# Kolkir/feature-point-cnn

Measured on AMD Instinct MI355X. Metric: frames/sec (VGA 640x480) SuperPoint fwd+NMS+descriptors, higher is better.
Workload: dtype f32

## Files before the change

### experiments/harness/w36_bench.hip

```cpp
#include <hip/hip_runtime.h>
#include <stdint.h>
#include <cmath>
#include <cstdio>
#include <cstdlib>
#include <cstring>
#include <random>
#include <vector>
#include <algorithm>
#include "../../feature-point-cnn_amd/csrc/wblock36_mfma.h"
using namespace fpc;
#define CK(x) do { hipError_t e_ = (x); if (e_ != hipSuccess) { printf("HIP error %s at line %d\n", hipGetErrorString(e_), __LINE__); exit(1);} } while (0)

static const double G43[6][3] = {{1.0 / 4, 0, 0}, {-1.0 / 6, -1.0 / 6, -1.0 / 6}, {-1.0 / 6, 1.0 / 6, -1.0 / 6},
                                 {1.0 / 24, 1.0 / 12, 1.0 / 6}, {1.0 / 24, -1.0 / 12, 1.0 / 6}, {0, 0, 1}};

struct Problem {
  int B, H, W, Cin, N, Cx;
  bool conv_only; int ysplit;
};

template <int NB, int TYT, int TXT>
static double run(const Problem& P, bool check, int reps, int grid_override = 0) {
  using C = W36Cfg<NB, TYT, TXT>;
  const int N = C::N, ncg = N / 16, nchunk = P.Cin / 16, nout = P.conv_only ? N * P.ysplit : N;
// ... 39 lines not shown
  float *dx, *dw1, *dw2, *db2, *dout;
  const size_t nout_el = (size_t)P.B * P.H * P.W * nout;
  CK(hipMalloc(&dx, x.size() * 4)); CK(hipMalloc(&dw1, w1p.size() * 4)); CK(hipMalloc(&dw2, w2p.size() * 4));
  CK(hipMalloc(&db2, N * 4)); CK(hipMalloc(&dout, nout_el * 4));
  CK(hipMemcpy(dx, x.data(), x.size() * 4, hipMemcpyHostToDevice));
  CK(hipMemcpy(dw1, w1p.data(), w1p.size() * 4, hipMemcpyHostToDevice));
  CK(hipMemcpy(dw2, w2p.data(), w2p.size() * 4, hipMemcpyHostToDevice));
  CK(hipMemcpy(db2, b2.data(), N * 4, hipMemcpyHostToDevice));
  CK(hipMemset(dout, 0xff, nout_el * 4));
  if (getenv("W36_PTRS")) printf("x %p..%p  w1 %p..%p  w2 %p..%p  b2 %p  out %p..%p\n", dx, dx + x.size(), dw1, dw1 + w1p.size(), dw2, dw2 + w2p.size(), db2, dout, dout + nout_el);
  WBlockArgs a{};
  a.x = dx; a.csx = P.Cin; a.nchunk = nchunk; a.H = P.H; a.W = P.W;
  a.w1 = (const float4*)dw1; a.b1 = dw1 + (size_t)ncg * gstride; a.w2 = (const float4*)dw2; a.b2 = db2;
  a.k8_h = k8_h; a.k8_x = k8_x; a.out = dout; a.cso = nout;
  a.tiles_x = (P.W + C::TW - 1) / C::TW; a.tiles_y = (P.H + C::TH - 1) / C::TH; a.frame0 = 0;
  a.total = a.tiles_x * a.tiles_y * P.B; a.xcd_order = 1; a.ysplit_floats = (int)half_floats;
  a.x_bytes = (unsigned)(x.size() * 4); a.conv_only = P.conv_only ? 1 : 0;
#ifdef FPC_DIAG
  unsigned long long* dst_; CK(hipMalloc(&dst_, 1024 * 8 * 8 + 1024 * 4 * 16 * 8)); CK(hipMemset(dst_, 0, 1024 * 8 * 8 + 1024 * 4 * 16 * 8)); a.stamps = dst_;
#endif
  CK(hipFuncSetAttribute((const void*)wblock36_kernel<NB, TYT, TXT>, hipFuncAttributeMaxDynamicSharedMemorySize, C::LDS_BYTES));
  int grid = grid_override ? grid_override : 256;
  if (grid > a.total) grid = a.total >= 8 ? (a.total / 8) * 8 : a.total;
  const dim3 g(grid, nh);
  hipLaunchKernelGGL((wblock36_kernel<NB, TYT, TXT>), g, dim3(256), C::LDS_BYTES, 0, a);
  CK(hipDeviceSynchronize());
  double result = 0;
  if (check) {
    std::vector<float> out(nout_el);
    CK(hipMemcpy(out.data(), dout, nout_el * 4, hipMemcpyDeviceToHost));
// ... 123 lines not shown
```

### experiments/harness/w36p_bench.hip

```cpp
#include <hip/hip_runtime.h>
#include <stdint.h>
#include <cmath>
#include <cstdio>
#include <cstdlib>
#include <cstring>
#include <random>
#include <vector>
#include <algorithm>
#include "../../feature-point-cnn_amd/csrc/wblock36p_mfma.h"
using namespace fpc;
#ifndef W36P_RING
#define W36P_RING 9
#endif
#define CK(x) do { hipError_t e_ = (x); if (e_ != hipSuccess) { printf("HIP error %s at line %d\n", hipGetErrorString(e_), __LINE__); exit(1);} } while (0)

static const double G43[6][3] = {{1.0 / 4, 0, 0}, {-1.0 / 6, -1.0 / 6, -1.0 / 6}, {-1.0 / 6, 1.0 / 6, -1.0 / 6},
                                 {1.0 / 24, 1.0 / 12, 1.0 / 6}, {1.0 / 24, -1.0 / 12, 1.0 / 6}, {0, 0, 1}};

struct Problem {
  int B, H, W, Cin, N, Cx;
  bool conv_only; int ysplit;
};

template <int NBP, int TYT, int TXT>
// ... 52 lines not shown
  float *dx, *dw1, *dw2, *db2, *dout;
  const size_t nout_el = (size_t)P.B * P.H * P.W * nout;
  CK(hipMalloc(&dx, x.size() * 4)); CK(hipMalloc(&dw1, w1p.size() * 4)); CK(hipMalloc(&dw2, w2p.size() * 4));
  CK(hipMalloc(&db2, N * 4)); CK(hipMalloc(&dout, nout_el * 4));
  CK(hipMemcpy(dx, x.data(), x.size() * 4, hipMemcpyHostToDevice));
  CK(hipMemcpy(dw1, w1p.data(), w1p.size() * 4, hipMemcpyHostToDevice));
  CK(hipMemcpy(dw2, w2p.data(), w2p.size() * 4, hipMemcpyHostToDevice));
  CK(hipMemcpy(db2, b2.data(), N * 4, hipMemcpyHostToDevice));
  CK(hipMemset(dout, 0xff, nout_el * 4));
  if (getenv("W36_PTRS")) printf("x %p..%p  w1 %p..%p  w2 %p..%p  b2 %p  out %p..%p\n", dx, dx + x.size(), dw1, dw1 + w1p.size(), dw2, dw2 + w2p.size(), db2, dout, dout + nout_el);
  WBlockArgs a{};
  a.x = dx; a.csx = P.Cin; a.nchunk = nchunk; a.H = P.H; a.W = P.W;
  a.w1 = (const float4*)dw1; a.b1 = dw1 + (size_t)ncg * gstride; a.w2 = (const float4*)dw2; a.b2 = db2;
  a.k8_h = k8_h; a.k8_x = k8_x; a.out = dout; a.cso = nout;
  a.tiles_x = (P.W + C::TW - 1) / C::TW; a.tiles_y = (P.H + C::TH - 1) / C::TH; a.frame0 = 0;
  a.total = a.tiles_x * a.tiles_y * P.B; a.xcd_order = 1; a.ysplit_floats = (int)half_floats;
  a.x_bytes = (unsigned)(x.size() * 4); a.conv_only = P.conv_only ? 1 : 0;
#ifdef FPC_DIAG
  unsigned long long* dst_; CK(hipMalloc(&dst_, 1024 * 8 * 8 + 1024 * 4 * 16 * 8)); CK(hipMemset(dst_, 0, 1024 * 8 * 8 + 1024 * 4 * 16 * 8)); a.stamps = dst_;
#endif
  CK(hipFuncSetAttribute(fn, hipFuncAttributeMaxDynamicSharedMemorySize, LDSB));
  int grid = grid_override ? grid_override : 256;
  if (grid > a.total) grid = a.total >= 8 ? (a.total / 8) * 8 : a.total;
  const dim3 g(grid, nh);
  launch(g, a);
  CK(hipDeviceSynchronize());
  double result = 0;
  if (check) {
    std::vector<float> out(nout_el);
    CK(hipMemcpy(out.data(), dout, nout_el * 4, hipMemcpyDeviceToHost));
// ... 120 lines not shown
```

### feature-point-cnn_amd/_lib.py

```python
import ctypes
import os
import subprocess

import torch

_DIR = os.path.dirname(os.path.abspath(__file__))
LIB_PATH = os.environ.get("FPC_LIB_PATH") or os.path.join(_DIR, "lib", "libfpc.so")
CSRC = os.path.join(_DIR, "csrc")

SYMBOLS = [
    "fpc_abi_version", "fpc_build_flags", "fpc_strerror", "fpc_last_hip_error", "fpc_default_config", "fpc_create",
    "fpc_destroy", "fpc_load_weights", "fpc_packed_size", "fpc_packed_device_ptr",
    "fpc_export_packed", "fpc_import_packed", "fpc_import_packed_device", "fpc_mark_weights_loaded", "fpc_set_stream", "fpc_upload_stream",
    "fpc_get_stream", "fpc_sync", "fpc_forward", "fpc_detect", "fpc_get_points", "fpc_results",
    "fpc_get_counts", "fpc_get_keypoints", "fpc_set_timing", "fpc_get_timings", "fpc_match", "fpc_first_within",
    "fpc_detect_u8", "fpc_u8_staging", "fpc_homography_adaptation", "fpc_detect_u8_resized",
    "fpc_sample_descriptors", "fpc_plan_hash", "fpc_broadcast_weights", "fpc_read_activation",
    "fpc_pack_layout_revision", "fpc_check_guards", "fpc_stream_report", "fpc_output_range",
    "fpc_match_frames", "fpc_first_within_frames",
    "fpc_default_ransac_params", "fpc_ransac_homography", "fpc_homography_frames",
    "fpc_bank_create", "fpc_bank_destroy", "fpc_bank_get", "fpc_bank_store", "fpc_bank_store_rows", "fpc_bank_clear",
    "fpc_match_bank", "fpc_homography_bank", "fpc_bank_create_ex", "fpc_bank_format",
    "fpc_match_frames_guided", "fpc_match_bank_guided",
    "fpc_cell_order", "fpc_match_frames_guided_cells", "fpc_match_bank_guided_cells",
    "fpc_bank_topk_reserve", "fpc_match_bank_topk", "fpc_homography_bank_topk",
    "fpc_ransac_fundamental", "fpc_fundamental_frames", "fpc_fundamental_bank",
    "fpc_match_frames_guided_epipolar", "fpc_match_bank_guided_epipolar",
]

ABI_VERSION = 4
PACK_LAYOUT_REVISION = 4

PLAN_FLAGS = {
    "no_fused_blocks": 1 << 0, "no_winograd": 1 << 1, "no_winograd_detector": 1 << 2, "no_winograd_layer_in1": 1 << 3,
    "no_xcd_order": 1 << 4, "no_fused_stem_pool": 1 << 5, "split_heads": 1 << 6, "nms_in_line": 1 << 7,
    "no_persistent_grid": 1 << 8, "layer1_tile_8x16": 1 << 9, "winograd_gen1": 1 << 10, "no_latency_tiles": 1 << 11,
    "nms_one_workgroup": 1 << 12, "no_fused_softmax": 1 << 13, "winograd_gen2": 1 << 14, "guard_zones": 1 << 15, "detector_gen1": 1 << 16, "heads_in_line": 1 << 17, "w36_one_wave": 1 << 18, "convt_phases": 1 << 19, "stem_round3": 1 << 20, "conv_round1": 1 << 21,
}


class FpcConfig(ctypes.Structure):
    _fields_ = [("device", ctypes.c_int), ("height", ctypes.c_int), ("width", ctypes.c_int),
                ("max_batch", ctypes.c_int), ("cell", ctypes.c_int), ("nms_dist", ctypes.c_int),
                ("conf_thresh", ctypes.c_float), ("border_remove", ctypes.c_int),
                ("descriptor_enabled", ctypes.c_int), ("max_keypoints", ctypes.c_int),
                ("in_channels", ctypes.c_int), ("dtype", ctypes.c_int), ("arch", ctypes.c_int),
                ("num_streams", ctypes.c_int), ("plan_flags", ctypes.c_uint), ("nms_round_launches", ctypes.c_int),
                ("min_sub_batch", ctypes.c_int)]


class FpcTensor(ctypes.Structure):
    _fields_ = [("name", ctypes.c_char_p), ("data", ctypes.c_void_p), ("ndim", ctypes.c_int),
# ... 159 lines not shown
```

### feature-point-cnn_amd/csrc/fpc_api.hip

```cpp
#include <hip/hip_runtime.h>

#include <dlfcn.h>

#include <algorithm>
#include <cmath>
#include <cstdio>
#include <cstdlib>
#include <cstring>
#include <memory>
#include <mutex>
#include <chrono>
#include <string>
#include <vector>

#include "../../include/fpc.h"
#include "block_mfma.h"
#include "block_bf16.h"
#include "convt_bf16.h"
#include "block_x3.h"
#include "stem_bf16.h"
#include "wblock_mfma.h"
#include "wblock16_mfma.h"
#include "wblock36_mfma.h"
#include "wblock36p_mfma.h"
// ... 281 lines not shown
   W36PCfg<TYT, TXT, true>::LDS_BYTES, 4, 4 * TYT, 4 * TXT, 512, (const void*)wblock36p_dust_kernel<TYT, TXT>, launchw_##name, true},
    FPC_W36PD_KINDS(X)
#undef X
};

static size_t w1_floats(const WKindInfo& k, int nchunk) {
  if (k.gen == 3) return (size_t)k.NCG * ((size_t)nchunk * 36 + (k.NCG == 8 ? W36Cfg<2, 4, 4>::WPAD : W36Cfg<1, 4, 4>::WPAD)) * 256;
  return (size_t)k.NCG * ((size_t)nchunk * 16 + W16Cfg<8>::WPAD) * 256;
}
static double wkind_mfma_flops(const WKindInfo& k, int tiles, int nchunk, int k8_1x1) {
  const double px = (double)k.TH * k.TW, n = k.NBT * 32.0;
  if (k.gen == 3) return 2.0 * tiles * n * (36.0 * (px / 16) * nchunk * k.KC + px * k8_1x1 * 8.0);
  return 2.0 * tiles * n * (16.0 * (px / 4) * nchunk * k.KC + px * k8_1x1 * 8.0);
}
static bool w36_fits(int , int H, int W, int cs_in, int cs_out) {
  return (unsigned long long)H * W * (unsigned long long)std::max(cs_in, cs_out) * sizeof(float) < (unsigned long long)W36_MARKER;
}
static int w36_frames_per_launch(int H, int W, int cs_in, int cs_out) {
  const unsigned long long fb = (unsigned long long)H * W * (unsigned long long)std::max(cs_in, cs_out) * sizeof(float);
  return (int)std::max<unsigned long long>(1, ((unsigned long long)W36_MARKER - 1) / fb);
}
static int w36_conv_part(int cout, int tiles, int cus) {
  if (cout < 128) return 64;
  if (cout == 128) return 128;
  const double t2 = std::ceil((double)tiles * (cout / 128) / cus) * 1.0, t1 = std::ceil((double)tiles * (cout / 64) / cus) * 0.53;
  return t1 < t2 ? 64 : 128;
}
static WKind w36_kind(int cout, int H, int W, bool paired = false) {
  const int t44 = ((H + 15) / 16) * ((W + 15) / 16), t28 = ((H + 7) / 8) * ((W + 31) / 32);
  if (cout == 65 && paired) return t28 < t44 ? WK_W36PD_C65_2x8 : WK_W36PD_C65_4x4;
  if (cout == 65) return t28 < t44 ? WK_W36_C65_2x8 : WK_W36_C65_4x4;
// ... 94 lines not shown
  int pH = 0, pW = 0, pC = 0;
  std::string prefix;
  int cin = 0, cout = 0;
  int grid_y = 1, grid_z = 1;
  double flops_per_frame = 0;
  double mfma_flops_per_frame = 0;
  bool fused_softmax_capable = false;
  double bytes_per_frame = 0;
  bool descriptor_branch = false;
};

struct Timing {
  hipEvent_t start, stop;
  int op;
  int frames;
};

}

using namespace fpc;

struct fpc_ctx {
  fpc_config cfg{};
  int H = 0, W = 0, B = 0, Hc = 0, Wc = 0;
  bool vgg = false;
  int D = 128;
  std::vector<float*> vbuf;
  size_t vconv0_off = 0;
  bool bf16 = false;
  bool split = false;
// ... 27 lines not shown
  bool nms_one_workgroup = false;
  int nms_g = 0;
  bool fuse_stem_pool = true;
  bool conv_lean = true;
  bool stem_lean = true;
  bool stem2 = false;
  bool layer1_t816 = false;
#ifdef FPC_DIAG
  unsigned long long* diag_stamps = nullptr;
  int diag_n = 0;
#endif
  bool winograd_in1 = true;
  bool winograd_det = true;
  int w36_cus = 0;
  bool w36_paired = true;
  bool winograd_det_gen3 = true;
  bool winograd = true;
  bool latency_tiles = true;
  int winograd_gen = 3;
  bool fuse_blocks = true;
  bool weights_loaded = false;
  bool plan_error = false;

  char* slab = nullptr;
  size_t slab_bytes = 0;
  bool guard_zones = false;
  std::vector<std::pair<size_t, size_t>> guards;
  float *stem_out, *x0, *h4, *x1, *x2, *h8, *x3, *cat, *dh, *dproj, *d0, *lg;
  float *h16, *y16a, *y16b, *lo_h, *lo0, *desc_map, *desc_in_nhwc;
  float* prob;
// ... 1823 lines not shown

struct Sub {
  int f0, n;
  bool small = false;
  bool fuse_softmax = false;
  hipStream_t st;
  hipStream_t side = nullptr;
  hipEvent_t ev_enc = nullptr, ev_det = nullptr;
};

struct LaunchTimer {
  fpc_ctx* c;
  int op;
  hipStream_t st;
  int frames;
  hipEvent_t s{}, e{};
  LaunchTimer(fpc_ctx* c_, int op_, hipStream_t st_, int frames_) : c(c_), op(op_), st(st_), frames(frames_) {
    if (c->timing) {
      s = next_event(c);
      e = next_event(c);
      hipEventRecord(s, st);
    }
  }
  ~LaunchTimer() {
    if (c->timing) {
      hipEventRecord(e, st);
      c->timings.push_back({s, e, op, frames});
    }
  }
};

static int op_index(const fpc_ctx* c, OpType t) {
  for (size_t i = 0; i < c->ops.size(); ++i)
    if (c->ops[i].type == t) return (int)i;
  return -1;
}

static void run_network(fpc_ctx* c, const float* frames, const Sub& sb0, int which, hipStream_t st) {
  Sub sb = sb0;
  sb.st = st;
  const int H = c->H, W = c->W, n = sb.n, f0 = sb.f0;
  for (size_t i = 0; i < c->ops.size(); ++i) {
// ... 78 lines not shown
      case OP_WBLOCK: {
        LaunchTimer t(c, (int)i, sb.st, n);
        WBlockArgs a = op.wargs;
        a.frame0 = f0;
#ifdef FPC_DIAG
        a.stamps = nullptr;
        if (const char* e = getenv("FPC_STAMP_OP"))
          if (op.name.find(e) != std::string::npos) {
            if (!c->diag_stamps) hipHostMalloc((void**)&c->diag_stamps, (size_t)65536 * 8 * sizeof(unsigned long long));
            memset(c->diag_stamps, 0, (size_t)65536 * 8 * sizeof(unsigned long long));
            a.stamps = c->diag_stamps;
            c->diag_n = a.tiles_x * a.tiles_y * n;
          }
#endif
        a.total = a.tiles_x * a.tiles_y * n;
        a.xcd_order = c->xcd_order ? 1 : 0;
        {
          const unsigned long long xb = (unsigned long long)(f0 + n) * a.H * a.W * a.csx * sizeof(float);
          a.x_bytes = xb > 0xfffffff0ull ? 0xfffffff0u : (unsigned)xb;
        }
        int grid = (c->persist_min_tiles > 0 && a.total >= c->persist_min_tiles * c->num_cus) ? c->num_cus : a.total;
        if (g_wkinds[op.wkind].gen == 3) {
          const int fpl = w36_frames_per_launch(a.H, a.W, a.csx, a.cso);
          const float* x0 = a.x;
          float* o0 = a.out;
          for (int g0 = 0; g0 < n; g0 += fpl) {
            const int gn = std::min(fpl, n - g0);
            a.frame0 = 0;
            a.x = x0 + (size_t)(f0 + g0) * a.H * a.W * a.csx;
            a.out = o0 + (size_t)(f0 + g0) * a.H * a.W * a.cso;
            a.total = a.tiles_x * a.tiles_y * gn;
            a.x_bytes = (unsigned)((unsigned long long)gn * a.H * a.W * a.csx * sizeof(float));
            const int cus_cap = c->w36_cus > 0 ? std::min(c->num_cus, c->w36_cus) : c->num_cus;
            const int cus8 = std::max(1, cus_cap / 8 / std::max(1, op.grid_y)), per_xcd = (a.total + 7) / 8;
            const int rounds = (per_xcd + cus8 - 1) / cus8;
            const int grid3 = 8 * std::min(cus8, (per_xcd + rounds - 1) / rounds);
            g_wkinds[op.wkind].launch(a, dim3(std::min(a.total, grid3), op.grid_y), sb.st);
          }
          break;
        }
        g_wkinds[op.wkind].launch(a, dim3(std::min(a.total, grid), op.grid_y), sb.st);
        break;
      }
      case OP_BLOCK: {
        LaunchTimer t(c, (int)i, sb.st, n);
        BlockArgs a = op.bargs;
        a.frame0 = f0;
#ifdef FPC_DIAG
        a.stamps = nullptr;
        if (const char* e = getenv("FPC_STAMP_OP"))
          if (op.name.find(e) != std::string::npos) {
            if (!c->diag_stamps) hipHostMalloc((void**)&c->diag_stamps, (size_t)65536 * 8 * sizeof(unsigned long long));
            memset(c->diag_stamps, 0, (size_t)65536 * 8 * sizeof(unsigned long long));
// ... 373 lines not shown
  const auto create_t0 = std::chrono::steady_clock::now();
  std::unique_lock<std::mutex> queue_lock(qmap::state().mu);
  const int probe_rounds0 = qmap::state().dev[cfg->device].rounds;
  c->stream = qmap::acquire(cfg->device, c.get(), SLOT_MAIN, true, qprobe, true);
  if (!c->stream) { qmap::release_owner(c.get()); g_hip_err = "hipStreamCreateWithFlags"; return FPC_E_HIP; }
  c->own_stream = true;
  {
    int nsub = cfg->num_streams > 0 ? std::min(8, cfg->num_streams) : (c->split ? 3 : 2);
    const unsigned pf = cfg->plan_flags;
    c->fuse_blocks = !(pf & FPC_PLAN_NO_FUSED_BLOCKS);
    c->guard_zones = (pf & FPC_PLAN_GUARD_ZONES) != 0;
    if (const char* e = getenv("FPC_GUARD_ZONES")) c->guard_zones = atoi(e) != 0;
    c->winograd_det_gen3 = !(pf & FPC_PLAN_DETECTOR_GEN1);
    c->w36_paired = !(pf & FPC_PLAN_W36_ONE_WAVE);
    if (const char* e = getenv("FPC_W36_PAIRED")) c->w36_paired = atoi(e) != 0;
    if (const char* e = getenv("FPC_W36_CUS")) c->w36_cus = std::max(0, atoi(e));
    if (const char* e = getenv("FPC_WINOGRAD_DET_GEN")) c->winograd_det_gen3 = atoi(e) >= 3;
    c->winograd = !(pf & FPC_PLAN_NO_WINOGRAD);
    c->winograd_det = !(pf & FPC_PLAN_NO_WINOGRAD_DETECTOR);
    c->winograd_in1 = !(pf & FPC_PLAN_NO_WINOGRAD_LAYER_IN1);
    c->xcd_order = !(pf & FPC_PLAN_NO_XCD_ORDER);
    c->fuse_stem_pool = !(pf & FPC_PLAN_NO_FUSED_STEM_POOL);
    c->stem_lean = !(pf & FPC_PLAN_STEM_ROUND3);
    c->conv_lean = !(pf & FPC_PLAN_CONV_ROUND1);
    if (const char* e = getenv("FPC_CONV_LEAN")) c->conv_lean = atoi(e) != 0;
    if (const char* e = getenv("FPC_STEM_LEAN")) c->stem_lean = atoi(e) != 0;
    c->split_heads = (pf & FPC_PLAN_SPLIT_HEADS) != 0;
    if (pf & FPC_PLAN_NO_PERSISTENT_GRID) c->persist_min_tiles = 0;
    c->layer1_t816 = (pf & FPC_PLAN_LAYER1_TILE_8x16) != 0;
    c->winograd_gen = (pf & FPC_PLAN_WINOGRAD_GEN1) ? 1 : (pf & FPC_PLAN_WINOGRAD_GEN2) ? 2 : 3;
// ... 1375 lines not shown
          case OP_CONV: k = op->lean ? lean_kind(op->kind)->symbol : g_kinds[op->kind].symbol; break;
          case OP_BLOCK: k = g_bkinds[op->bkind].symbol; break;
          case OP_WBLOCK: k = g_wkinds[op->wkind].symbol; break;
          case OP_BF16: k = g_fkinds[op->fkind].symbol; break;
          case OP_SOFTMAX: k = "softmax_d2s_kernel"; break;
          case OP_NMS: k = c->nms_one_workgroup ? "nms_rounds_kernel+nms_sort_kernel" : "nms_rounds_kernel+nms_finish_kernel+nms_chunk_sort_kernel+nms_merge_kernel"; break;
          case OP_DESC: k = "descriptor16_kernel"; break;
          case OP_VCONV0: k = "vgg_conv0_kernel"; break;
          case OP_POOL2: k = "maxpool2_kernel"; break;
          case OP_L2NORM: k = "l2norm256_kernel"; break;
        }
      kernels[i] = k;
    }
    if (ms) ms[i] = v;
    if (flops) flops[i] = op ? op->flops_per_frame * t.frames : 0.0;
    if (mfma_flops) mfma_flops[i] = op ? op->mfma_flops_per_frame * t.frames : 0.0;
    if (bytes) bytes[i] = op ? op->bytes_per_frame * t.frames : 0.0;
  }
  return n;
}

}
```

### feature-point-cnn_amd/csrc/wblock36_mfma.h

```cpp
#pragma once
#include <type_traits>
#include <utility>

#include "wblock16_mfma.h"

namespace fpc {

template <int... I, class F>
__device__ __forceinline__ void fpc_static_for_impl(std::integer_sequence<int, I...>, F&& f) {
  (f(std::integral_constant<int, I>{}), ...);
}
template <int N, class F>
__device__ __forceinline__ void fpc_static_for(F&& f) {
  fpc_static_for_impl(std::make_integer_sequence<int, N>{}, f);
}

struct W36Dust {
  static constexpr int W2ROW = 0, W2COL = 64, WPCOL = 144, B1 = 400, B2 = 401, UIN64 = 404, UIN = 448, UOUT = 448 + 4 * 36 * 16;
  static constexpr int floats(int nchunk) { return UOUT + nchunk * 36 * 16; }
};

template <int NB_, int TYT_, int TXT_, bool DUST_ = false>
struct W36Cfg {
  static constexpr int NB = NB_, TYT = TYT_, TXT = TXT_;
// ... 67 lines not shown
  "v_mfma_f32_16x16x4_f32 %2, %9, %21, %2\n\tv_mfma_f32_16x16x4_f32 %3, %9, %25, %3\n\t"                               \
  "v_mfma_f32_16x16x4_f32 %0, %6, %14, %0\n\tv_mfma_f32_16x16x4_f32 %1, %6, %18, %1\n\t"                               \
  "v_mfma_f32_16x16x4_f32 %2, %10, %22, %2\n\tv_mfma_f32_16x16x4_f32 %3, %10, %26, %3\n\t"                             \
  "v_mfma_f32_16x16x4_f32 %0, %7, %15, %0\n\tv_mfma_f32_16x16x4_f32 %1, %7, %19, %1\n\t"                               \
  "v_mfma_f32_16x16x4_f32 %2, %11, %23, %2\n\tv_mfma_f32_16x16x4_f32 %3, %11, %27, %3"
#define FPC_MFMA16_IN                                                                                                   \
  "v"(a0[0]), "v"(a0[1]), "v"(a0[2]), "v"(a0[3]), "v"(a1[0]), "v"(a1[1]), "v"(a1[2]), "v"(a1[3]), "v"(b00[0]), "v"(b00[1]), \
      "v"(b00[2]), "v"(b00[3]), "v"(b01[0]), "v"(b01[1]), "v"(b01[2]), "v"(b01[3]), "v"(b10[0]), "v"(b10[1]), "v"(b10[2]),  \
      "v"(b10[3]), "v"(b11[0]), "v"(b11[1]), "v"(b11[2]), "v"(b11[3])
  if constexpr (AG) asm volatile(FPC_MFMA16 : "+a"(c00), "+a"(c01), "+a"(c10), "+a"(c11) : FPC_MFMA16_IN);
  else asm volatile(FPC_MFMA16 : "+v"(c00), "+v"(c01), "+v"(c10), "+v"(c11) : FPC_MFMA16_IN);
#undef FPC_MFMA16
#undef FPC_MFMA16_IN
}

template <int NB, int TYT, int TXT, bool DUST>
__device__ __forceinline__ void wblock36_body(const WBlockArgs& a) {
  using C = W36Cfg<NB, TYT, TXT, DUST>;
  constexpr int NT = C::NT, TH = C::TH, TW = C::TW, HW = C::HW, HH = C::HH, HROW = C::HROW, HIT = C::HIT;
  constexpr int N = C::N, RH = C::RH, RX = C::RX, RING = C::RING, STEPS = C::STEPS, HPX = C::HPX;
  extern __shared__ __attribute__((aligned(16))) float lds[];
  f32x4* const lds4 = reinterpret_cast<f32x4*>(lds);
  constexpr int TL4 = C::OFF_H0 / 4;

  const int tid = threadIdx.x, lane = tid & 63;
  const unsigned lane16 = (unsigned)lane * 16u;
  const int wave = __builtin_amdgcn_readfirstlane(tid >> 6);
  const int tiles = a.tiles_x * a.tiles_y;
  const int nchunk = a.nchunk;
  const float4* const w1h = a.w1 + (size_t)blockIdx.y * (a.ysplit_floats / 4);
  const float* const b1h = a.b1 + (size_t)blockIdx.y * a.ysplit_floats;

  const bool xcd_order = a.xcd_order && (gridDim.x & 7) == 0;
  const int wg_step = xcd_order ? (int)(gridDim.x >> 3) : (int)gridDim.x;
  const int xchunk = (a.total + 7) >> 3;
  const int wg_first = xcd_order ? (int)(blockIdx.x & 7) * xchunk + (int)(blockIdx.x >> 3) : (int)blockIdx.x;
  const int wg_end = xcd_order ? min(a.total, ((int)(blockIdx.x & 7) + 1) * xchunk) : a.total;
  if (wg_first >= wg_end) return;

  const __amdgpu_buffer_rsrc_t xrsrc = __builtin_amdgcn_make_buffer_rsrc(const_cast<float*>(a.x), 0, (int)a.x_bytes, 0x00020000);
  int okoff[HIT];
  int okoff64[DUST ? C::HIT64 : 1];
  struct TilePos { int b, ty, tx, live; };
  auto tile_pos = [&](int wg) {
    TilePos q;
    q.live = wg < wg_end;
    const int wgc = q.live ? wg : wg_first;
    const int bl = wgc / tiles;
    const int t = wgc - bl * tiles;
    q.b = a.frame0 + bl;
    q.ty = t / a.tiles_x;
    q.tx = t - q.ty * a.tiles_x;
    return q;
  };
  auto halo_base = [&](const TilePos& q) {
    return __builtin_amdgcn_readfirstlane(((q.b * a.H + q.ty * TH) * a.W + q.tx * TW) * a.csx * 4);
  };
  auto halo_tile = [&](const TilePos& q) {
    int tl = tid;
    asm volatile("" : "+v"(tl));
    const int iy0 = q.ty * TH - 1, ix0 = q.tx * TW - 1;
    const int hlim = q.live ? a.H : 0;
#pragma unroll
    for (int i = 0; i < HIT; ++i) {
      const int e = tl + i * NT;
      const int pix = (e * 13108) >> 16, c4 = e - pix * 5;
      const int hy = HW == 18 ? (pix * 3641) >> 16 : (pix * 1928) >> 16;
      const int hx = pix - hy * HW;
      const bool ok = ((unsigned)(iy0 + hy) < (unsigned)hlim) & ((unsigned)(ix0 + hx) < (unsigned)a.W) & (hy < HH) & (c4 < 4);
      const int off = (((hy - 1) * a.W + (hx - 1)) * a.csx + c4 * 4) * 4;
      okoff[i] = ok ? off : W36_MARKER;
    }
    if constexpr (DUST) {
#pragma unroll
      for (int i = 0; i < C::HIT64; ++i) {
        const int pix = tl + i * NT;
        const int hy = HW == 18 ? (pix * 3641) >> 16 : (pix * 1928) >> 16;
        const int hx = pix - hy * HW;
        const bool ok = ((unsigned)(iy0 + hy) < (unsigned)hlim) & ((unsigned)(ix0 + hx) < (unsigned)a.W) & (hy < HH) & (a.dust_in != 0);
        okoff64[i] = ok ? (((hy - 1) * a.W + (hx - 1)) * a.csx + 64) * 4 : W36_MARKER;
      }
    }
  };
  auto load_halo = [&](int base, int hoff) {
#pragma unroll
    for (int i = 0; i < HIT; ++i) {
      int voff;
      asm("v_add_i32 %0, %1, %2 clamp" : "=v"(voff) : "v"(okoff[i]), "s"(base));
      __builtin_amdgcn_raw_ptr_buffer_load_lds(xrsrc, (__attribute__((address_space(3))) void*)(lds + hoff + (i * NT + wave * 64) * 4), 16, voff, 0, 0, 0);
    }
  };
  auto load_halo64 = [&](int base) {
    if constexpr (DUST) {
#pragma unroll
      for (int i = 0; i < C::HIT64; ++i) {
// ... 74 lines not shown
  if constexpr (DUST) {
    d_va = wave * 64 + lane;
    d_ua = wave * 64 + 16 * ((lane & 3) ^ (2 * (lane >> 5)));
    for (int i = tid; i < 448 / 4; i += NT) lds4[C::D_HEAD / 4 + i] = reinterpret_cast<const f32x4*>(a.dust)[i];
    for (int i = tid; i < 2304 / 4; i += NT) lds4[C::D_UIN / 4 + i] = reinterpret_cast<const f32x4*>(a.dust + W36Dust::UIN)[i];
  }

  TilePos pos_cur = tile_pos(wg_first);
  int base_cur = halo_base(pos_cur);
  halo_tile(pos_cur);
  load_halo64(base_cur);
  load_halo(base_cur, C::OFF_H0);
  load_halo(base_cur + 64, C::OFF_H1);
  asm volatile("s_waitcnt vmcnt(%0)" ::"n"(HIT) : "memory");
  FPC_LDS_BARRIER();
  transform_all(C::OFF_H0, C::OFF_V0);
  FPC_LDS_BARRIER();

  constexpr int C4 = N / 4, EIT = HPX * C4 / NT, PPI = NT / C4;
  constexpr int CPR = TW / PPI;
  const __amdgpu_buffer_rsrc_t orsrc = __builtin_amdgcn_make_buffer_rsrc(a.out + blockIdx.y * N, 0, W36_MARKER, 0x00020000);

  const int g2s = __builtin_amdgcn_readfirstlane(((a.k8_h + a.k8_x) / 2 + C::WPAD2) * 64);
  const __amdgpu_buffer_rsrc_t w2rsrc = __builtin_amdgcn_make_buffer_rsrc(const_cast<float4*>(a.w2), 0, a.conv_only ? 0 : 4 * NB * g2s * 16, 0x00020000);
  const unsigned w2lane = (unsigned)(wave * NB * g2s) * 16u + lane16;

  const int wg_stamp = wg_first + 2 * wg_step < wg_end ? wg_first + 2 * wg_step : wg_first;
  for (int wg = wg_first; wg < wg_end; wg += wg_step) {
    const int b = pos_cur.b, ty = pos_cur.ty, tx = pos_cur.tx;
    const TilePos pos_next = tile_pos(wg + wg_step);
    const int base_next = halo_base(pos_next);
    if (wg == wg_stamp) { FPC_STAMP(0) FPC_RSTAMP(6) }

    f32x4 acc[36][NB];
    {
      float zf = 0.f;
      asm volatile("" : "+v"(zf));
#pragma unroll
      for (int p = 0; p < 36; ++p)
#pragma unroll
        for (int nb = 0; nb < NB; ++nb) acc[p][nb] = f32x4{zf, zf, zf, zf};
    }

    BF bq[RING];
// ... 2 lines not shown
    if constexpr (DUST) {
      float zf = 0.f;
      asm volatile("" : "+v"(zf));
#pragma unroll
      for (int i = 0; i < 9; ++i) dacc[i] = zf;
    }

    auto chunk_body = [&](auto PAR, const int c) {
      constexpr int par = decltype(PAR)::value;
      constexpr int VB_OFF = par ? C::OFF_V1 : C::OFF_V0, VN_OFF = par ? C::OFF_V0 : C::OFF_V1;
      constexpr int HS_OFF = par ? C::OFF_H1 : C::OFF_H0;
      constexpr int HN_OFF = par ? C::OFF_H0 : C::OFF_H1;
      const int c3 = c + 2;
      const bool nxt = c3 >= nchunk;
      const int l_base = (nxt ? base_next : base_cur) + (nxt ? c3 - nchunk : c3) * 64;
      int ao = aoff4 + VB_OFF / 4, trd_c = trd + HN_OFF, twr_c = twr + VN_OFF;
      asm volatile("" : "+v"(ao), "+v"(trd_c), "+v"(twr_c));
      [[maybe_unused]] int dva = d_va + VB_OFF / 4;
      [[maybe_unused]] f32x4 dv[3];
      if constexpr (DUST) asm volatile("" : "+v"(dva));
      constexpr int AQ = 2;
      f32x4 ac[2][AQ];
#pragma unroll
      for (int q = 0; q < AQ; ++q) ac[0][q] = lds4[ao + q * 64];
#ifdef FPC_DIAG_STEPS
      unsigned long long tq[11] = {0, 0, 0, 0, 0, 0, 0, 0, 0, 0, 0};
#define FPC_TQ(i) asm volatile("s_memtime %0" : "=s"(tq[i]));
#else
#define FPC_TQ(i)
#endif
      fpc_static_for<STEPS>([&](auto S) __attribute__((always_inline)) {
// ... 78 lines not shown
      do {
        chunk_body(std::integral_constant<int, 0>{}, c);
        chunk_body(std::integral_constant<int, 1>{}, c + 1);
        c += 2;
      } while (c < nchunk);
    }
    if (wg == wg_stamp) { FPC_STAMP(1) }
    asm volatile("s_nop 15\n\ts_nop 7" ::: "memory");

    if constexpr (DUST) {
      int tid_d = tid;
      asm volatile("" : "+v"(tid_d));
      const int lane_d = tid_d & 63;
      if (a.dust_in) {
        if (tid_d < 16) {
          const int rd = C::D_H64 + ((4 * (tid_d / TXT)) * HW + 4 * (tid_d % TXT)) * 4;
#pragma unroll
          for (int i = 0; i < 6; ++i)
#pragma unroll
            for (int j = 0; j < 6; ++j) tp[i][j >> 1][j & 1] = lds[rd + (i * HW + j) * 4];
          t_burst();
          const int mrow = ((tid_d & 7) >> 1) * 4 + (tid_d >> 3) * 2 + (tid_d & 1);
#pragma unroll
          for (int i = 0; i < 6; ++i)
#pragma unroll
            for (int j = 0; j < 6; ++j) lds[C::D_V64 + (i * 6 + j) * 16 + mrow] = tp[2 * (i >> 1) + (j & 1)][j >> 1][i & 1];
        }
        FPC_LDS_BARRIER();
        {
          const int va = C::D_V64 + (lane_d & 15), ub = C::D_UIN + wave * 576 + (lane_d & 15);
          float av[36], bv[36];
// ... 141 lines not shown
          }
        }
      }
      }
    }
    __builtin_amdgcn_sched_barrier(0);

    const int m0 = tid_t / C4, c4t = tid_t - m0 * C4;
    const int opart = (m0 * a.cso + c4t * 4) * 4;
    int ocol[CPR];
#pragma unroll
    for (int k = 0; k < CPR; ++k) ocol[k] = (tx * TW + m0 + k * PPI < a.W) ? opart + k * PPI * a.cso * 4 : W36_MARKER;

#pragma unroll
    for (int half = 0; half < 2; ++half) {
      const int y0 = ty * TH + half * (TH / 2), x0 = tx * TW;
      const int rows_valid = min(TH / 2, a.H - y0);
      const int xbase = __builtin_amdgcn_readfirstlane(((b * a.H + y0) * a.W + x0) * a.csx * 4);
      const int obase = __builtin_amdgcn_readfirstlane(((b * a.H + y0) * a.W + x0) * a.cso * 4);
      if (half == 1) {
#pragma unroll
        for (int nb = 0; nb < NB; ++nb)
#pragma unroll
          for (int rr = 0; rr < 2; ++rr)
#pragma unroll
            for (int i = 0; i < 4; ++i)
#pragma unroll
              for (int jj = 0; jj < 4; ++jj) lds[hw_base[rr] + 16 * nb + (i * TW + jj) * RH] = yh1[nb][rr][i * 4 + jj];
        if constexpr (DUST) {
          const int T = 8 * ((tid_t >> 1) & 1) + 2 * (tid_t >> 2) + (tid_t & 1), th = T & 7;
          if (tid_t < 16 && T >= 8) {
            const int hb = C::OFF_H0 + ((4 * (th / TXT)) * TW + 4 * (th % TXT)) * RH + 64;
#pragma unroll
            for (int i = 0; i < 4; ++i)
// ... 236 lines not shown
```

### feature-point-cnn_amd/csrc/wblock_mfma.h

```cpp
#pragma once
#include "block_mfma.h"

namespace fpc {

struct WBlockArgs {
  const float* x;
  int csx, nchunk;
  int H, W;
  const float4* w1;
  const float* b1;
  const float4* w2;
  const float* b2;
  int k8_h, k8_x;
  float* out;
  int cso, tiles_x, tiles_y, frame0;
  int total;
  int xcd_order;
  int ysplit_floats;
  unsigned x_bytes;
  int conv_only;
  const float* dust;
  int dust_in;
#ifdef FPC_DIAG
  unsigned long long* stamps;
#endif
};

template <int KC, int NBT, int CMID_>
struct WBlockCfg {
  static constexpr int TH = 8, TW = 16, NT = 512;
  static constexpr int HW = TW + 2, HH = TH + 2;
  static constexpr int ROW4 = KC / 4 + 1;
  static constexpr int CMID = CMID_;
  static constexpr int ROWH4 = CMID / 4 + 1;
  static constexpr int HALO_BYTES = HH * HW * ROW4 * 16;
  static constexpr int V_BYTES = 16 * 32 * ROW4 * 16;
  static constexpr int M_BYTES = 16 * 32 * 36 * 4;
// ... 408 lines not shown
```

### include/fpc.h

```cpp
#ifndef FPC_H
#define FPC_H

#include <stddef.h>
#include <stdint.h>

#ifdef __cplusplus
extern "C" {
#endif

#define FPC_ABI_VERSION 4
#define FPC_PACK_LAYOUT_REVISION 4

enum {
  FPC_OK = 0,
  FPC_E_INVALID = -1,
  FPC_E_NO_DEVICE = -2,
  FPC_E_HIP = -3,
  FPC_E_NO_WEIGHTS = -4,
  FPC_E_MISSING_KEY = -5,
  FPC_E_CAPACITY = -6,
  FPC_E_NOT_CONVERGED = -7,
  FPC_E_RANGE = -8,
  FPC_E_NONFINITE = -9
};
// ... 28 lines not shown
  FPC_PLAN_NO_WINOGRAD_LAYER_IN1 = 1 << 3,
  FPC_PLAN_NO_XCD_ORDER = 1 << 4,
  FPC_PLAN_NO_FUSED_STEM_POOL = 1 << 5,
  FPC_PLAN_SPLIT_HEADS = 1 << 6,
  FPC_PLAN_NMS_IN_LINE = 1 << 7,
  FPC_PLAN_NO_PERSISTENT_GRID = 1 << 8,
  FPC_PLAN_LAYER1_TILE_8x16 = 1 << 9,
  FPC_PLAN_WINOGRAD_GEN1 = 1 << 10,
  FPC_PLAN_NO_LATENCY_TILES = 1 << 11,
  FPC_PLAN_NMS_ONE_WORKGROUP = 1 << 12,
  FPC_PLAN_NO_FUSED_SOFTMAX = 1 << 13,
  FPC_PLAN_WINOGRAD_GEN2 = 1 << 14,
  FPC_PLAN_HEADS_IN_LINE = 1 << 17,
  FPC_PLAN_DETECTOR_GEN1 = 1 << 16,
  FPC_PLAN_W36_ONE_WAVE = 1 << 18,
  FPC_PLAN_STEM_ROUND3 = 1 << 20,
  FPC_PLAN_CONV_ROUND1 = 1 << 21,
  FPC_PLAN_CONVT_PHASES = 1 << 19,
  FPC_PLAN_GUARD_ZONES = 1 << 15
};

typedef struct fpc_tensor {
  const char* name;
  const float* data;
  int ndim;
  int64_t shape[4];
} fpc_tensor;

typedef struct fpc_device_results {
  const int32_t* count;
// ... 176 lines not shown
```

Baseline: 12120.

## Stack frames vertically in W36 Winograd block to avoid partial edge tiles

When frame height is not a multiple of the 16-row tile, the W36 fused Winograd block now treats a batch of frames as one tall image. Tiles that straddle a frame boundary load a split halo with a gap row, so padding stays correct at the seam. This removes the partially empty bottom tile of each frame and cuts the total tile count. In exchange the halo-address math gains a per-tile boundary shift, a reciprocal divide and extra predicates. The path is on by default and can be disabled with a plan flag or environment variable.

Result: no change. 12220, median of 6 (+0.8%).

```diff
diff --git a/experiments/harness/w36_bench.hip b/experiments/harness/w36_bench.hip
--- a/experiments/harness/w36_bench.hip
+++ b/experiments/harness/w36_bench.hip
@@ -77,6 +77,7 @@
   a.w1 = (const float4*)dw1; a.b1 = dw1 + (size_t)ncg * gstride; a.w2 = (const float4*)dw2; a.b2 = db2;
   a.k8_h = k8_h; a.k8_x = k8_x; a.out = dout; a.cso = nout;
   a.tiles_x = (P.W + C::TW - 1) / C::TW; a.tiles_y = (P.H + C::TH - 1) / C::TH; a.frame0 = 0;
+  a.stack_rows = P.H; a.h_rcp = (unsigned)((0x100000000ull + P.H - 1) / P.H);
   a.total = a.tiles_x * a.tiles_y * P.B; a.xcd_order = 1; a.ysplit_floats = (int)half_floats;
   a.x_bytes = (unsigned)(x.size() * 4); a.conv_only = P.conv_only ? 1 : 0;
 #ifdef FPC_DIAG
diff --git a/experiments/harness/w36p_bench.hip b/experiments/harness/w36p_bench.hip
--- a/experiments/harness/w36p_bench.hip
+++ b/experiments/harness/w36p_bench.hip
@@ -90,6 +90,7 @@
   a.w1 = (const float4*)dw1; a.b1 = dw1 + (size_t)ncg * gstride; a.w2 = (const float4*)dw2; a.b2 = db2;
   a.k8_h = k8_h; a.k8_x = k8_x; a.out = dout; a.cso = nout;
   a.tiles_x = (P.W + C::TW - 1) / C::TW; a.tiles_y = (P.H + C::TH - 1) / C::TH; a.frame0 = 0;
+  a.stack_rows = P.H; a.h_rcp = (unsigned)((0x100000000ull + P.H - 1) / P.H);
   a.total = a.tiles_x * a.tiles_y * P.B; a.xcd_order = 1; a.ysplit_floats = (int)half_floats;
   a.x_bytes = (unsigned)(x.size() * 4); a.conv_only = P.conv_only ? 1 : 0;
 #ifdef FPC_DIAG
diff --git a/feature-point-cnn_amd/_lib.py b/feature-point-cnn_amd/_lib.py
--- a/feature-point-cnn_amd/_lib.py
+++ b/feature-point-cnn_amd/_lib.py
@@ -36,6 +36,7 @@
     "no_xcd_order": 1 << 4, "no_fused_stem_pool": 1 << 5, "split_heads": 1 << 6, "nms_in_line": 1 << 7,
     "no_persistent_grid": 1 << 8, "layer1_tile_8x16": 1 << 9, "winograd_gen1": 1 << 10, "no_latency_tiles": 1 << 11,
     "nms_one_workgroup": 1 << 12, "no_fused_softmax": 1 << 13, "winograd_gen2": 1 << 14, "guard_zones": 1 << 15, "detector_gen1": 1 << 16, "heads_in_line": 1 << 17, "w36_one_wave": 1 << 18, "convt_phases": 1 << 19, "stem_round3": 1 << 20, "conv_round1": 1 << 21,
+    "w36_per_frame": 1 << 22,
 }
 
 
diff --git a/feature-point-cnn_amd/csrc/fpc_api.hip b/feature-point-cnn_amd/csrc/fpc_api.hip
--- a/feature-point-cnn_amd/csrc/fpc_api.hip
+++ b/feature-point-cnn_amd/csrc/fpc_api.hip
@@ -319,7 +319,12 @@
   return 2.0 * tiles * n * (16.0 * (px / 4) * nchunk * k.KC + px * k8_1x1 * 8.0);
 }
 static bool w36_fits(int , int H, int W, int cs_in, int cs_out) {
+  if (H >= 32768 || W >= 32768) return false;
   return (unsigned long long)H * W * (unsigned long long)std::max(cs_in, cs_out) * sizeof(float) < (unsigned long long)W36_MARKER;
+}
+static bool w36_stacks(const WKindInfo& k, bool enabled, int H, int frames) {
+  return enabled && k.gen == 3 && k.TH == 16 && k.threads == 256 && !k.dust && H % 4 == 0 && H >= 12 && H % 16 != 0 && frames > 1 &&
+         (unsigned long long)frames * H * H < 0x100000000ull;
 }
 static int w36_frames_per_launch(int H, int W, int cs_in, int cs_out) {
   const unsigned long long fb = (unsigned long long)H * W * (unsigned long long)std::max(cs_in, cs_out) * sizeof(float);
@@ -444,6 +449,7 @@
   hipEvent_t start, stop;
   int op;
   int frames;
+  double mfma_flops = -1.0;
 };
 
 }
@@ -501,6 +507,7 @@
   bool winograd_det = true;
   int w36_cus = 0;
   bool w36_paired = true;
+  bool w36_stack = true;
   bool winograd_det_gen3 = true;
   bool winograd = true;
   bool latency_tiles = true;
@@ -2354,6 +2361,7 @@
   int op;
   hipStream_t st;
   int frames;
+  double mfma_flops = -1.0;
   hipEvent_t s{}, e{};
   LaunchTimer(fpc_ctx* c_, int op_, hipStream_t st_, int frames_) : c(c_), op(op_), st(st_), frames(frames_) {
     if (c->timing) {
@@ -2365,7 +2373,7 @@
   ~LaunchTimer() {
     if (c->timing) {
       hipEventRecord(e, st);
-      c->timings.push_back({s, e, op, frames});
+      c->timings.push_back({s, e, op, frames, mfma_flops});
     }
   }
 };
@@ -2474,6 +2482,8 @@
           }
 #endif
         a.total = a.tiles_x * a.tiles_y * n;
+        a.stack_rows = a.H;
+        a.h_rcp = 0;
         a.xcd_order = c->xcd_order ? 1 : 0;
         {
           const unsigned long long xb = (unsigned long long)(f0 + n) * a.H * a.W * a.csx * sizeof(float);
@@ -2484,12 +2494,18 @@
           const int fpl = w36_frames_per_launch(a.H, a.W, a.csx, a.cso);
           const float* x0 = a.x;
           float* o0 = a.out;
+          int tiles_run = 0;
           for (int g0 = 0; g0 < n; g0 += fpl) {
             const int gn = std::min(fpl, n - g0);
             a.frame0 = 0;
             a.x = x0 + (size_t)(f0 + g0) * a.H * a.W * a.csx;
             a.out = o0 + (size_t)(f0 + g0) * a.H * a.W * a.cso;
-            a.total = a.tiles_x * a.tiles_y * gn;
+            const bool stack = w36_stacks(g_wkinds[op.wkind], c->w36_stack, a.H, gn);
+            a.stack_rows = stack ? gn * a.H : a.H;
+            a.h_rcp = (unsigned)((0x100000000ull + a.H - 1) / a.H);
+            a.tiles_y = (a.stack_rows + g_wkinds[op.wkind].TH - 1) / g_wkinds[op.wkind].TH;
+            a.total = a.tiles_x * a.tiles_y * (stack ? 1 : gn);
+            tiles_run += a.total;
             a.x_bytes = (unsigned)((unsigned long long)gn * a.H * a.W * a.csx * sizeof(float));
             const int cus_cap = c->w36_cus > 0 ? std::min(c->num_cus, c->w36_cus) : c->num_cus;
             const int cus8 = std::max(1, cus_cap / 8 / std::max(1, op.grid_y)), per_xcd = (a.total + 7) / 8;
@@ -2497,6 +2513,10 @@
             const int grid3 = 8 * std::min(cus8, (per_xcd + rounds - 1) / rounds);
             g_wkinds[op.wkind].launch(a, dim3(std::min(a.total, grid3), op.grid_y), sb.st);
           }
+          t.mfma_flops = op.mfma_flops_per_frame * tiles_run / (op.wargs.tiles_x * op.wargs.tiles_y);
+#ifdef FPC_DIAG
+          if (a.stamps) c->diag_n = tiles_run;
+#endif
           break;
         }
         g_wkinds[op.wkind].launch(a, dim3(std::min(a.total, grid), op.grid_y), sb.st);
@@ -2900,6 +2920,8 @@
     c->winograd_det_gen3 = !(pf & FPC_PLAN_DETECTOR_GEN1);
     c->w36_paired = !(pf & FPC_PLAN_W36_ONE_WAVE);
     if (const char* e = getenv("FPC_W36_PAIRED")) c->w36_paired = atoi(e) != 0;
+    c->w36_stack = !(pf & FPC_PLAN_W36_PER_FRAME);
+    if (const char* e = getenv("FPC_W36_STACK")) c->w36_stack = atoi(e) != 0;
     if (const char* e = getenv("FPC_W36_CUS")) c->w36_cus = std::max(0, atoi(e));
     if (const char* e = getenv("FPC_WINOGRAD_DET_GEN")) c->winograd_det_gen3 = atoi(e) >= 3;
     c->winograd = !(pf & FPC_PLAN_NO_WINOGRAD);
@@ -4305,7 +4327,7 @@
     }
     if (ms) ms[i] = v;
     if (flops) flops[i] = op ? op->flops_per_frame * t.frames : 0.0;
-    if (mfma_flops) mfma_flops[i] = op ? op->mfma_flops_per_frame * t.frames : 0.0;
+    if (mfma_flops) mfma_flops[i] = !op ? 0.0 : t.mfma_flops >= 0 ? t.mfma_flops : op->mfma_flops_per_frame * t.frames;
     if (bytes) bytes[i] = op ? op->bytes_per_frame * t.frames : 0.0;
   }
   return n;
diff --git a/feature-point-cnn_amd/csrc/wblock36_mfma.h b/feature-point-cnn_amd/csrc/wblock36_mfma.h
--- a/feature-point-cnn_amd/csrc/wblock36_mfma.h
+++ b/feature-point-cnn_amd/csrc/wblock36_mfma.h
@@ -105,6 +105,44 @@
 #undef FPC_MFMA16_IN
 }
 
+struct W36Tile {
+  int row0, span_tx, top_bnd;
+  __device__ __forceinline__ int span() const { return span_tx & 0xffff; }
+  __device__ __forceinline__ int tx() const { return span_tx >> 16; }
+  __device__ __forceinline__ int top() const { return top_bnd & 0xffff; }
+  __device__ __forceinline__ int bnd() const { return top_bnd >> 16; }
+  __device__ __forceinline__ int hi() const { return row0 - top() + span(); }
+};
+constexpr int W36_NO_BND = 64;
+
+template <int TH, bool STACKABLE>
+__device__ __forceinline__ W36Tile w36_tile(const WBlockArgs& a, int tiles, int wgc, int live) {
+  W36Tile q;
+  const int bl = wgc / tiles;
+  const int t = wgc - bl * tiles;
+  const int ty = t / a.tiles_x;
+  const int tx = t - ty * a.tiles_x;
+  const int r0 = ty * TH;
+  int top, span, bnd;
+  if constexpr (STACKABLE) {
+    const int fh = (int)__umulhi((unsigned)r0, a.h_rcp) * a.H;
+    const int nb = fh + a.H;
+    const bool in = nb < min(r0 + TH, a.stack_rows);
+    q.row0 = a.frame0 * a.H + bl * a.stack_rows + r0;
+    top = r0 - fh;
+    span = in ? 2 * a.H : a.H;
+    bnd = in ? nb - r0 : W36_NO_BND;
+  } else {
+    q.row0 = (a.frame0 + bl) * a.H + r0;
+    top = r0;
+    span = a.H;
+    bnd = W36_NO_BND;
+  }
+  q.span_tx = (live ? span : 0) | (tx << 16);
+  q.top_bnd = top | (bnd << 16);
+  return q;
+}
+
 template <int NB, int TYT, int TXT, bool DUST>
 __device__ __forceinline__ void wblock36_body(const WBlockArgs& a) {
   using C = W36Cfg<NB, TYT, TXT, DUST>;
@@ -132,34 +170,33 @@
   const __amdgpu_buffer_rsrc_t xrsrc = __builtin_amdgcn_make_buffer_rsrc(const_cast<float*>(a.x), 0, (int)a.x_bytes, 0x00020000);
   int okoff[HIT];
   int okoff64[DUST ? C::HIT64 : 1];
-  struct TilePos { int b, ty, tx, live; };
+  using TilePos = W36Tile;
+  constexpr bool STACKABLE = TYT == 4 && !DUST;
   auto tile_pos = [&](int wg) {
-    TilePos q;
-    q.live = wg < wg_end;
-    const int wgc = q.live ? wg : wg_first;
-    const int bl = wgc / tiles;
-    const int t = wgc - bl * tiles;
-    q.b = a.frame0 + bl;
-    q.ty = t / a.tiles_x;
-    q.tx = t - q.ty * a.tiles_x;
-    return q;
+    const int live = wg < wg_end;
+    return w36_tile<TH, STACKABLE>(a, tiles, live ? wg : wg_first, live);
   };
   auto halo_base = [&](const TilePos& q) {
-    return __builtin_amdgcn_readfirstlane(((q.b * a.H + q.ty * TH) * a.W + q.tx * TW) * a.csx * 4);
+    return __builtin_amdgcn_readfirstlane((q.row0 * a.W + q.tx() * TW) * a.csx * 4);
   };
+  auto halo_shift = [&](const TilePos& q, int gy4) { return STACKABLE && gy4 >= q.bnd() ? 1 : 0; };
   auto halo_tile = [&](const TilePos& q) {
     int tl = tid;
     asm volatile("" : "+v"(tl));
-    const int iy0 = q.ty * TH - 1, ix0 = q.tx * TW - 1;
-    const int hlim = q.live ? a.H : 0;
+    W36Tile u = q;
+    asm volatile("" : "+s"(u.span_tx), "+s"(u.top_bnd));
+    const int iy0 = u.top() - 1, ix0 = u.tx() * TW - 1;
+    const int hlim = u.span(), qbnd = STACKABLE ? u.bnd() : W36_NO_BND;
+    const int hyn = HH + (qbnd < TH ? 1 : 0), gap = qbnd + 1;
 #pragma unroll
     for (int i = 0; i < HIT; ++i) {
       const int e = tl + i * NT;
       const int pix = (e * 13108) >> 16, c4 = e - pix * 5;
       const int hy = HW == 18 ? (pix * 3641) >> 16 : (pix * 1928) >> 16;
       const int hx = pix - hy * HW;
-      const bool ok = ((unsigned)(iy0 + hy) < (unsigned)hlim) & ((unsigned)(ix0 + hx) < (unsigned)a.W) & (hy < HH) & (c4 < 4);
-      const int off = (((hy - 1) * a.W + (hx - 1)) * a.csx + c4 * 4) * 4;
+      const int hr = hy - (hy > qbnd ? 1 : 0);
+      const bool ok = ((unsigned)(iy0 + hr) < (unsigned)hlim) & ((unsigned)(ix0 + hx) < (unsigned)a.W) & (hy < hyn) & (hy != gap) & (c4 < 4);
+      const int off = (((hr - 1) * a.W + (hx - 1)) * a.csx + c4 * 4) * 4;
       okoff[i] = ok ? off : W36_MARKER;
     }
     if constexpr (DUST) {
@@ -168,8 +205,9 @@
         const int pix = tl + i * NT;
         const int hy = HW == 18 ? (pix * 3641) >> 16 : (pix * 1928) >> 16;
         const int hx = pix - hy * HW;
-        const bool ok = ((unsigned)(iy0 + hy) < (unsigned)hlim) & ((unsigned)(ix0 + hx) < (unsigned)a.W) & (hy < HH) & (a.dust_in != 0);
-        okoff64[i] = ok ? (((hy - 1) * a.W + (hx - 1)) * a.csx + 64) * 4 : W36_MARKER;
+        const int hr = hy - (hy > qbnd ? 1 : 0);
+        const bool ok = ((unsigned)(iy0 + hr) < (unsigned)hlim) & ((unsigned)(ix0 + hx) < (unsigned)a.W) & (hy < hyn) & (hy != gap) & (a.dust_in != 0);
+        okoff64[i] = ok ? (((hr - 1) * a.W + (hx - 1)) * a.csx + 64) * 4 : W36_MARKER;
       }
     }
   };
@@ -274,7 +312,7 @@
   load_halo(base_cur + 64, C::OFF_H1);
   asm volatile("s_waitcnt vmcnt(%0)" ::"n"(HIT) : "memory");
   FPC_LDS_BARRIER();
-  transform_all(C::OFF_H0, C::OFF_V0);
+  transform_all(C::OFF_H0 + halo_shift(pos_cur, 4 * wave) * (HW * HROW), C::OFF_V0);
   FPC_LDS_BARRIER();
 
   constexpr int C4 = N / 4, EIT = HPX * C4 / NT, PPI = NT / C4;
@@ -287,7 +325,7 @@
 
   const int wg_stamp = wg_first + 2 * wg_step < wg_end ? wg_first + 2 * wg_step : wg_first;
   for (int wg = wg_first; wg < wg_end; wg += wg_step) {
-    const int b = pos_cur.b, ty = pos_cur.ty, tx = pos_cur.tx;
+    const int row0 = pos_cur.row0, row_hi = pos_cur.hi(), tx = pos_cur.tx();
     const TilePos pos_next = tile_pos(wg + wg_step);
     const int base_next = halo_base(pos_next);
     if (wg == wg_stamp) { FPC_STAMP(0) FPC_RSTAMP(6) }
@@ -320,7 +358,8 @@
       const int c3 = c + 2;
       const bool nxt = c3 >= nchunk;
       const int l_base = (nxt ? base_next : base_cur) + (nxt ? c3 - nchunk : c3) * 64;
-      int ao = aoff4 + VB_OFF / 4, trd_c = trd + HN_OFF, twr_c = twr + VN_OFF;
+      const int tsh = halo_shift(c + 1 < nchunk ? pos_cur : pos_next, 4 * wave) * (HW * HROW);
+      int ao = aoff4 + VB_OFF / 4, trd_c = trd + (HN_OFF + tsh), twr_c = twr + VN_OFF;
       asm volatile("" : "+v"(ao), "+v"(trd_c), "+v"(twr_c));
       [[maybe_unused]] int dva = d_va + VB_OFF / 4;
       [[maybe_unused]] f32x4 dv[3];
@@ -429,7 +468,8 @@
       const int lane_d = tid_d & 63;
       if (a.dust_in) {
         if (tid_d < 16) {
-          const int rd = C::D_H64 + ((4 * (tid_d / TXT)) * HW + 4 * (tid_d % TXT)) * 4;
+          const int gy4 = 4 * (tid_d / TXT);
+          const int rd = C::D_H64 + ((gy4 + halo_shift(pos_cur, gy4)) * HW + 4 * (tid_d % TXT)) * 4;
 #pragma unroll
           for (int i = 0; i < 6; ++i)
 #pragma unroll
@@ -601,10 +641,10 @@
 
 #pragma unroll
     for (int half = 0; half < 2; ++half) {
-      const int y0 = ty * TH + half * (TH / 2), x0 = tx * TW;
-      const int rows_valid = min(TH / 2, a.H - y0);
-      const int xbase = __builtin_amdgcn_readfirstlane(((b * a.H + y0) * a.W + x0) * a.csx * 4);
-      const int obase = __builtin_amdgcn_readfirstlane(((b * a.H + y0) * a.W + x0) * a.cso * 4);
+      const int y0 = row0 + half * (TH / 2), x0 = tx * TW;
+      const int rows_valid = min(TH / 2, row_hi - y0);
+      const int xbase = __builtin_amdgcn_readfirstlane((y0 * a.W + x0) * a.csx * 4);
+      const int obase = __builtin_amdgcn_readfirstlane((y0 * a.W + x0) * a.cso * 4);
       if (half == 1) {
 #pragma unroll
         for (int nb = 0; nb < NB; ++nb)
diff --git a/feature-point-cnn_amd/csrc/wblock_mfma.h b/feature-point-cnn_amd/csrc/wblock_mfma.h
--- a/feature-point-cnn_amd/csrc/wblock_mfma.h
+++ b/feature-point-cnn_amd/csrc/wblock_mfma.h
@@ -21,6 +21,8 @@
   int conv_only;
   const float* dust;
   int dust_in;
+  int stack_rows;
+  unsigned h_rcp;
 #ifdef FPC_DIAG
   unsigned long long* stamps;
 #endif
diff --git a/include/fpc.h b/include/fpc.h
--- a/include/fpc.h
+++ b/include/fpc.h
@@ -66,6 +66,7 @@
   FPC_PLAN_HEADS_IN_LINE = 1 << 17,
   FPC_PLAN_DETECTOR_GEN1 = 1 << 16,
   FPC_PLAN_W36_ONE_WAVE = 1 << 18,
+  FPC_PLAN_W36_PER_FRAME = 1 << 22,
   FPC_PLAN_STEM_ROUND3 = 1 << 20,
   FPC_PLAN_CONV_ROUND1 = 1 << 21,
   FPC_PLAN_CONVT_PHASES = 1 << 19,
```
